# malb/m4ri

Measured on AMD Instinct MI355X. Metric: gf2_matmul_n3_equiv_bitops_per_sec, higher is better.
Workload: dtype u64; 1 GPU; mzd_mul 65536x65536x65536 (BASELINE.json configs[2]/[3]): Strassen-Winograd levels, the fused bottom ones by a rank-47 scheme of the 4 x 4 x 4 block product, over M4RM leaves; m=65536, l=65536, n=65536, input=splitmix64 seeds 3 (A), 4 (B), uniform bits, resident in HBM, strassen_levels=4, leaf_products_per_rank=2209, parallelism=1 GPU

## Files before the change

### m4ri_amd/csrc/scheme444.h

```cpp
#pragma once
#include <stdint.h>
#define SCHEME444_R 47
static constexpr uint16_t SCHEME444_U[SCHEME444_R] = {0x0101, 0x0808, 0x0d0d, 0x0e0e, 0x1000, 0x1001, 0x1010, 0x1110, 0x2d32, 0x3d32, 0x3d38, 0x3d3d, 0x3d3e, 0x5d08, 0x5d38, 0x5d58, 0x5d98, 0x6798, 0x6868, 0x6d38, 0x6e08, 0x7798, 0x8000, 0x8008, 0x8088, 0x8888, 0x9198, 0x9798, 0x9898, 0x9d98, 0xbd38, 0xcd01, 0xcd32, 0xcd98, 0xcdcd, 0xd000, 0xdd00, 0xddd0, 0xdddd, 0xe000, 0xe0e0, 0xe0ee, 0xee00, 0xf1fe, 0xf798, 0xfd32, 0xfe01};
static constexpr uint16_t SCHEME444_V[SCHEME444_R] = {0x0111, 0x1100, 0x0110, 0x0010, 0x0333, 0x0a14, 0xb1ac, 0xe7f9, 0x0927, 0x0777, 0x7700, 0x0a10, 0x0e10, 0xb1a0, 0x00f0, 0x7160, 0x0fff, 0x0aaa, 0x7760, 0x0aa0, 0xeef0, 0xe4ca, 0x3300, 0x4e50, 0x819f, 0xd7ca, 0xe1ff, 0x0060, 0xb1aa, 0x0660, 0x7d50, 0x011f, 0x00b0, 0xbb00, 0x0117, 0x0330, 0xb1af, 0x7e60, 0x0a17, 0x0030, 0x7d60, 0x0917, 0xe4fa, 0x0717, 0xee00, 0x0ee0, 0x0a1a};
static constexpr uint16_t SCHEME444_W[SCHEME444_R] = {0xbe5b, 0xb66b, 0xb1a0, 0xb158, 0xee0e, 0xbe5e, 0xbb0b, 0xbb5b, 0x4eae, 0x4ea4, 0xc66c, 0xb1a7, 0xb15f, 0xb6d0, 0xc628, 0xb11b, 0x0ee0, 0x8e68, 0xb16b, 0xc6a0, 0xb658, 0x8868, 0x6666, 0xb6b6, 0xbbbb, 0xbb6b, 0xb55b, 0x8268, 0xbd6b, 0x0aa0, 0xc6c6, 0xbe50, 0x4ea8, 0x0660, 0xb1ab, 0xa0a0, 0xb0b0, 0xb1b1, 0xb1a1, 0x28c8, 0xb1c1, 0xb151, 0xb858, 0xb15b, 0x8668, 0x4ea0, 0xbe58};
```

### m4ri_amd/csrc/scheme_passes.hip

```cpp
#include <hip/hip_runtime.h>
#include <cstdlib>
#include "gf2_internal.h"
#include "scheme444.h"

namespace {

constexpr int R444 = SCHEME444_R;

struct Tables { uint16_t m[3][3][50]; };
constexpr Tables make_tables() {
  Tables t{};
  constexpr uint16_t WG[3][7] = {{0x1, 0x2, 0xF, 0x8, 0xC, 0xD, 0x5}, {0x1, 0x4, 0x8, 0xF, 0x3, 0xB, 0xA}, {0xF, 0x1, 0x2, 0x4, 0xA, 0xE, 0xC}};
  for (int side = 0; side < 3; ++side) {
    t.m[0][side][0] = 1;
    for (int r = 0; r < 7; ++r) t.m[1][side][r] = WG[side][r];
    for (int r = 0; r < R444; ++r) t.m[2][side][r] = side == 0 ? SCHEME444_U[r] : side == 1 ? SCHEME444_V[r] : SCHEME444_W[r];
  }
  return t;
}
__constant__ Tables c_tab = make_tables();

struct Outer { int32_t r1, lv, side; };
__device__ __forceinline__ uint32_t outer_mask(const Outer &o, int r1) { return (uint32_t)c_tab.m[o.lv][o.side][r1]; }

template <int POS>
__device__ __forceinline__ uint32_t wave_union(uint32_t mine) {
  if (POS == 64) return __builtin_amdgcn_readfirstlane(mine);
  return __builtin_amdgcn_readfirstlane(mine) | __builtin_amdgcn_readlane(mine, 32);
}

template <int G, int POS>
__device__ __forceinline__ void form_top(const word *grid, uint32_t mine, int pp, word (&x)[16]) {
  constexpr int GD = 4 * G;
  const uint32_t both = wave_union<POS>(mine);
#pragma unroll
  for (int f = 0; f < 16; ++f) x[f] = 0;
#pragma unroll 1
  for (int c = 0; c < G * G; ++c) {
    if (!((both >> c) & 1)) continue;
    const word keep = (POS == 64 || ((mine >> c) & 1)) ? ~(word)0 : 0;
    const int i1 = c / G, j1 = c % G;
#pragma unroll
    for (int f = 0; f < 16; ++f) x[f] ^= grid[((4 * i1 + (f >> 2)) * GD + 4 * j1 + (f & 3)) * POS + pp] & keep;
  }
}

template <bool BSIDE>
__device__ __forceinline__ word inner_child(const word (&x)[16], int r2) {
  const uint16_t m = BSIDE ? SCHEME444_V[r2] : SCHEME444_U[r2];
  word v = 0;
#pragma unroll
  for (int f = 0; f < 16; ++f)
    if ((m >> f) & 1) v ^= x[f];
  return v;
}

template <int G, int POS, int UNITS, bool BSIDE>
__global__ __launch_bounds__(POS * UNITS) void scheme_down_kernel(const word *__restrict__ anc, int64_t p_stride, int64_t p_bs,
                                   word *__restrict__ child, int64_t c_bs,
                                   int64_t crows, int64_t cw, Outer o) {
  constexpr int GD = 4 * G, NB = GD * GD;
  __shared__ word grid[NB * POS];
  constexpr int units = UNITS;
  const int tid = threadIdx.x, pp = tid % POS, unit = tid / POS;
  const int64_t i = (int64_t)blockIdx.x * POS + pp, pi = blockIdx.y;
  const int64_t r = i / cw, w = i - r * cw;
  const word *p = anc + pi * p_bs + r * p_stride + w;
#pragma unroll 8
  for (int k = 0; k < (NB + UNITS - 1) / UNITS; ++k) {
    const int blk = k * UNITS + unit;
    if (NB % UNITS == 0 || blk < NB) grid[blk * POS + pp] = p[(int64_t)(blk / GD) * crows * p_stride + (int64_t)(blk % GD) * cw];
  }
  __syncthreads();
  word *out = child + pi * (int64_t)o.r1 * R444 * c_bs + r * cw + w;
  for (int r0 = 0; r0 < o.r1; r0 += units) {
    const int r1 = r0 + unit;
    const uint32_t mine = r1 < o.r1 ? outer_mask(o, r1) : 0u;
    word x[16];
    form_top<G, POS>(grid, mine, pp, x);
    if (r1 >= o.r1) continue;
    word *q = out + (int64_t)r1 * R444 * c_bs;
#pragma unroll
    for (int r2 = 0; r2 < R444; ++r2) q[(int64_t)r2 * c_bs] = inner_child<BSIDE>(x, r2);
  }
}

template <int G, int POS, int UNITS>
__global__ __launch_bounds__(POS * UNITS) void scheme_down_pack_kernel(const word *__restrict__ anc, int64_t p_stride, int64_t p_bs,
                                        uint32_t *__restrict__ a4, int64_t a4_bs,
                                        int64_t crows, int64_t cw, Outer o) {
  constexpr int GD = 4 * G, NB = GD * GD;
  __shared__ word grid[NB * POS];
  constexpr int units = UNITS;
  const int tid = threadIdx.x, pp = tid % POS, unit = tid / POS;
  const int64_t b = blockIdx.x, grp = b >> 7, xcd = b & 7, slot = (b >> 3) & 15;
  const int64_t wgroups = cw >> 4;
  const int64_t rb = (grp / wgroups) * 8 + xcd, wc = (grp % wgroups) * 16 + slot;
  if (rb * POS >= crows) return;
  const int64_t r = rb * POS + pp, pi = blockIdx.y;
  const word *p = anc + pi * p_bs + r * p_stride + wc;
#pragma unroll 8
  for (int k = 0; k < (NB + UNITS - 1) / UNITS; ++k) {
    const int blk = k * UNITS + unit;
    if (NB % UNITS == 0 || blk < NB) grid[blk * POS + pp] = p[(int64_t)(blk / GD) * crows * p_stride + (int64_t)(blk % GD) * cw];
  }
  __syncthreads();
  const uint32_t rot = (uint32_t)((r >> 6) & 3);
  uint32_t *out = a4 + pi * (int64_t)o.r1 * R444 * a4_bs + (2 * wc) * crows + r;
  for (int r0 = 0; r0 < o.r1; r0 += units) {
    const int r1 = r0 + unit;
    const uint32_t mine = r1 < o.r1 ? outer_mask(o, r1) : 0u;
    word x[16];
    form_top<G, POS>(grid, mine, pp, x);
    if (r1 >= o.r1) continue;
    uint32_t *q = out + (int64_t)r1 * R444 * a4_bs;
#pragma unroll
    for (int r2 = 0; r2 < R444; ++r2) {
      const word v = inner_child<false>(x, r2);
      uint32_t w0 = (uint32_t)v, w1 = (uint32_t)(v >> 32);
      w0 = __builtin_amdgcn_alignbyte(w0, w0, rot);
      w1 = __builtin_amdgcn_alignbyte(w1, w1, rot);
      uint32_t *oo = q + (int64_t)r2 * a4_bs;
      oo[0]     = w0;
      oo[crows] = w1;
    }
  }
}

template <int G, int POS, int UNITS, bool ACC>
__global__ __launch_bounds__(POS * UNITS) void scheme_up_kernel(const word *__restrict__ prod, int64_t p_bs,
                                 word *anc, int64_t o_stride, int64_t o_bs, int64_t crows, int64_t cw, Outer o) {
  constexpr int GD = 4 * G, NB = GD * GD;
  __shared__ unsigned long long g[NB * POS];
  constexpr int units = UNITS;
  const int tid = threadIdx.x, pp = tid % POS, unit = tid / POS;
  for (int k = tid; k < NB * POS; k += POS * UNITS) g[k] = 0;
  __syncthreads();
  const int64_t i = (int64_t)blockIdx.x * POS + pp, pi = blockIdx.y;
  const int64_t r = i / cw, w = i - r * cw;
  const word *q0 = prod + pi * (int64_t)o.r1 * R444 * p_bs + r * cw + w;
  for (int r1 = unit; r1 < o.r1; r1 += units) {
    const word *q = q0 + (int64_t)r1 * R444 * p_bs;
    word y[16];
#pragma unroll
    for (int f = 0; f < 16; ++f) y[f] = 0;
#pragma unroll
    for (int g0 = 0; g0 < R444; g0 += 8) {
      word v[8];
#pragma unroll
      for (int k = 0; k < 8; ++k)
        if (g0 + k < R444) v[k] = q[(int64_t)(g0 + k) * p_bs];
#pragma unroll
      for (int k = 0; k < 8; ++k)
        if (g0 + k < R444) {
          const uint16_t m = SCHEME444_W[g0 + k];
#pragma unroll
          for (int f = 0; f < 16; ++f)
            if ((m >> f) & 1) y[f] ^= v[k];
        }
    }
    const uint32_t mine = outer_mask(o, r1);
#pragma unroll 1
    for (int c = 0; c < G * G; ++c) {
      if (!((mine >> c) & 1)) continue;
      const int i1 = c / G, k1 = c % G;
#pragma unroll
      for (int f = 0; f < 16; ++f) atomicXor(&g[((4 * i1 + (f >> 2)) * GD + 4 * k1 + (f & 3)) * POS + pp], (unsigned long long)y[f]);
    }
  }
  __syncthreads();
  word *out = anc + pi * o_bs + r * o_stride + w;
#pragma unroll 4
  for (int k = 0; k < (NB + UNITS - 1) / UNITS; ++k) {
    const int blk = k * UNITS + unit;
    if (NB % UNITS != 0 && blk >= NB) continue;
    word *oo     = out + (int64_t)(blk / GD) * crows * o_stride + (int64_t)(blk % GD) * cw;
    const word v = g[blk * POS + pp];
    *oo          = ACC ? (*oo ^ v) : v;
  }
}

Outer outer_for(int levels, int side) { return Outer{levels == 4 ? R444 : levels == 3 ? 7 : 1, levels - 2, side}; }

constexpr int64_t MAX_GRID_Y = 65535;
constexpr int POS_B = 64;

}

extern "C" int gf2_scheme444_rank(void) { return R444; }

extern "C" int64_t gf2_scheme444_leaves(int levels) { return levels == 4 ? (int64_t)R444 * R444 : levels == 3 ? 7 * (int64_t)R444 : levels == 2 ? R444 : 0; }

extern "C" int gf2_scheme444_ok(int levels, int64_t a_rows, int64_t a_cw, int64_t b_rows, int64_t b_cw) {
  static const int sw = getenv("M4RI_AMD_SCHEME") ? atoi(getenv("M4RI_AMD_SCHEME")) : -1;
  if (sw == 0 || (sw == 4 && levels != 4) || (sw < 0 && R444 >= 49)) return 0;
  if (levels < 2 || levels > 4) return 0;
  if (a_rows <= 0 || b_rows <= 0 || a_rows % (levels == 2 ? 64 : 32) != 0 || a_cw % 16 != 0 || b_cw % POS_B != 0) return 0;
  if ((a_rows * a_cw) / 2 > 0x7fffffffLL || (b_rows * b_cw) / 32 > 0x7fffffffLL || (a_rows * b_cw) / 32 > 0x7fffffffLL) return 0;
  return 1;
}

template <typename F>
static void with_inner_grid(int levels, F &&f) {
  if (levels == 4) f(std::integral_constant<int, 4>{});
  else if (levels == 3) f(std::integral_constant<int, 2>{});
  else f(std::integral_constant<int, 1>{});
}

extern "C" hipError_t gf2_launch_scheme_down(hipStream_t s, int levels, int bside, const word *anc, int64_t p_stride, int64_t p_bs, word *child,
                                             int64_t nparents, int64_t crows, int64_t cw) {
  const int64_t c_bs = crows * cw;
  if (nparents * c_bs == 0) return hipSuccess;
  if (levels < 2 || levels > 4 || cw % 64 != 0) return hipErrorInvalidValue;
  const Outer o = outer_for(levels, bside ? 1 : 0);
  const int64_t leaves = gf2_scheme444_leaves(levels);
  for (int64_t p0 = 0; p0 < nparents; p0 += MAX_GRID_Y) {
    const int64_t np = nparents - p0 < MAX_GRID_Y ? nparents - p0 : MAX_GRID_Y;
    const word *an = anc + p0 * p_bs;
    word *ch       = child + p0 * leaves * c_bs;
    const dim3 g((unsigned)(c_bs / 64), (unsigned)np);
    with_inner_grid(levels, [&](auto G_) {
      constexpr int G = decltype(G_)::value, UNITS = G == 4 ? 8 : G == 2 ? 7 : 1;
      with_bool(bside, [&](auto BS) {
        hipLaunchKernelGGL((scheme_down_kernel<G, 64, UNITS, decltype(BS)::value>), g, dim3(64 * UNITS), 0, s, an, p_stride, p_bs, ch, c_bs, crows, cw, o);
      });
    });
  }
  return hipGetLastError();
}

extern "C" hipError_t gf2_launch_scheme_down_pack(hipStream_t s, int levels, const word *anc, int64_t p_stride, int64_t p_bs, word *a4,
                                                  int64_t nparents, int64_t crows, int64_t cw) {
  if (nparents * crows * cw == 0) return hipSuccess;
  const int pos = levels == 2 ? 64 : 32;
  if (levels < 2 || levels > 4 || crows % pos != 0 || cw % 16 != 0) return hipErrorInvalidValue;
  const Outer o = outer_for(levels, 0);
  const int64_t groups = ((crows / pos + 7) / 8) * (cw / 16);
  if (groups * 128 > 0x7fffffffLL) return hipErrorInvalidValue;
  const int64_t leaves = gf2_scheme444_leaves(levels);
  for (int64_t p0 = 0; p0 < nparents; p0 += MAX_GRID_Y) {
    const int64_t np = nparents - p0 < MAX_GRID_Y ? nparents - p0 : MAX_GRID_Y;
    const word *an = anc + p0 * p_bs;
    uint32_t *pk   = reinterpret_cast<uint32_t *>(a4) + p0 * leaves * crows * cw * 2;
    const dim3 g((unsigned)(groups * 128), (unsigned)np);
    with_inner_grid(levels, [&](auto G_) {
      constexpr int G = decltype(G_)::value, POS = G == 1 ? 64 : 32, UNITS = G == 1 ? 1 : 8;
      hipLaunchKernelGGL((scheme_down_pack_kernel<G, POS, UNITS>), g, dim3(POS * UNITS), 0, s, an, p_stride, p_bs, pk, crows * cw * 2, crows, cw, o);
    });
  }
  return hipGetLastError();
}

extern "C" hipError_t gf2_launch_scheme_up(hipStream_t s, int levels, int acc, const word *prod, word *anc, int64_t o_stride, int64_t o_bs,
                                           int64_t nparents, int64_t crows, int64_t cw) {
  const int64_t p_bs = crows * cw;
  if (nparents * p_bs == 0) return hipSuccess;
  if (levels < 2 || levels > 4 || cw % 64 != 0) return hipErrorInvalidValue;
  const Outer o = outer_for(levels, 2);
  const int pos = levels == 2 ? 64 : 32;
  const int64_t leaves = gf2_scheme444_leaves(levels);
  for (int64_t p0 = 0; p0 < nparents; p0 += MAX_GRID_Y) {
    const int64_t np = nparents - p0 < MAX_GRID_Y ? nparents - p0 : MAX_GRID_Y;
    const word *pr = prod + p0 * leaves * p_bs;
    word *an       = anc + p0 * o_bs;
    const dim3 g((unsigned)(p_bs / pos), (unsigned)np);
    with_inner_grid(levels, [&](auto G_) {
      constexpr int G = decltype(G_)::value, POS = G == 1 ? 64 : 32, UNITS = G == 1 ? 1 : 8;
      with_bool(acc, [&](auto ACC) {
        hipLaunchKernelGGL((scheme_up_kernel<G, POS, UNITS, decltype(ACC)::value>), g, dim3(POS * UNITS), 0, s, pr, p_bs, an, o_stride, o_bs, crows, cw, o);
      });
    });
  }
  return hipGetLastError();
}
```

Baseline: 11330000 billion bit-op/s.

## Use common-subexpression XOR programs for 4x4x4 scheme and wave-uniform outer loops

Replaces the naive per-output XOR accumulation of the rank-47 U, V and W^T maps with precomputed straight-line XOR programs that share intermediate sums. This cuts the XOR count in the down and up passes. The outer-rank loops are made wave-uniform and iterate only the set bits of the outer mask, which removes the wave-union masking. For POS=32, the pack and up kernels switch to 32-bit lanes so a full wave covers each block. The restructured lane/chunk addressing adds complexity and some correctness risk.

New measurement: 11380000 billion bit-op/s (median of 6 runs). No clear change (+0.4%).

```diff
diff --git a/m4ri_amd/csrc/scheme444.h b/m4ri_amd/csrc/scheme444.h
--- a/m4ri_amd/csrc/scheme444.h
+++ b/m4ri_amd/csrc/scheme444.h
@@ -4,3 +4,458 @@
 static constexpr uint16_t SCHEME444_U[SCHEME444_R] = {0x0101, 0x0808, 0x0d0d, 0x0e0e, 0x1000, 0x1001, 0x1010, 0x1110, 0x2d32, 0x3d32, 0x3d38, 0x3d3d, 0x3d3e, 0x5d08, 0x5d38, 0x5d58, 0x5d98, 0x6798, 0x6868, 0x6d38, 0x6e08, 0x7798, 0x8000, 0x8008, 0x8088, 0x8888, 0x9198, 0x9798, 0x9898, 0x9d98, 0xbd38, 0xcd01, 0xcd32, 0xcd98, 0xcdcd, 0xd000, 0xdd00, 0xddd0, 0xdddd, 0xe000, 0xe0e0, 0xe0ee, 0xee00, 0xf1fe, 0xf798, 0xfd32, 0xfe01};
 static constexpr uint16_t SCHEME444_V[SCHEME444_R] = {0x0111, 0x1100, 0x0110, 0x0010, 0x0333, 0x0a14, 0xb1ac, 0xe7f9, 0x0927, 0x0777, 0x7700, 0x0a10, 0x0e10, 0xb1a0, 0x00f0, 0x7160, 0x0fff, 0x0aaa, 0x7760, 0x0aa0, 0xeef0, 0xe4ca, 0x3300, 0x4e50, 0x819f, 0xd7ca, 0xe1ff, 0x0060, 0xb1aa, 0x0660, 0x7d50, 0x011f, 0x00b0, 0xbb00, 0x0117, 0x0330, 0xb1af, 0x7e60, 0x0a17, 0x0030, 0x7d60, 0x0917, 0xe4fa, 0x0717, 0xee00, 0x0ee0, 0x0a1a};
 static constexpr uint16_t SCHEME444_W[SCHEME444_R] = {0xbe5b, 0xb66b, 0xb1a0, 0xb158, 0xee0e, 0xbe5e, 0xbb0b, 0xbb5b, 0x4eae, 0x4ea4, 0xc66c, 0xb1a7, 0xb15f, 0xb6d0, 0xc628, 0xb11b, 0x0ee0, 0x8e68, 0xb16b, 0xc6a0, 0xb658, 0x8868, 0x6666, 0xb6b6, 0xbbbb, 0xbb6b, 0xb55b, 0x8268, 0xbd6b, 0x0aa0, 0xc6c6, 0xbe50, 0x4ea8, 0x0660, 0xb1ab, 0xa0a0, 0xb0b0, 0xb1b1, 0xb1a1, 0x28c8, 0xb1c1, 0xb151, 0xb858, 0xb15b, 0x8668, 0x4ea0, 0xbe58};
+
+#if defined(__HIPCC__)
+#define SCHEME444_FN __host__ __device__ __forceinline__
+#else
+#define SCHEME444_FN inline
+#endif
+
+#define SCHEME444_XORS_U 82
+template <typename T, typename Emit> SCHEME444_FN void scheme444_apply_u(const T (&x)[16], Emit &&emit) {
+  const T t16 = x[0] ^ x[8];
+  emit(0, t16);
+  const T t17 = x[3] ^ x[11];
+  emit(1, t17);
+  const T t18 = x[10] ^ x[11];
+  const T t19 = x[3] ^ t18;
+  const T t20 = x[0] ^ x[2];
+  const T t21 = x[8] ^ t20;
+  const T t22 = t19 ^ t21;
+  emit(2, t22);
+  const T t23 = x[1] ^ x[2];
+  const T t24 = t19 ^ t23;
+  const T t25 = x[9] ^ t24;
+  emit(3, t25);
+  emit(4, x[12]);
+  const T t26 = x[0] ^ x[12];
+  emit(5, t26);
+  const T t27 = x[4] ^ x[12];
+  emit(6, t27);
+  const T t28 = x[4] ^ x[8];
+  const T t29 = x[12] ^ t28;
+  emit(7, t29);
+  const T t30 = x[5] ^ x[13];
+  const T t31 = t28 ^ t30;
+  const T t32 = x[1] ^ t18;
+  const T t33 = t31 ^ t32;
+  emit(8, t33);
+  const T t34 = t29 ^ t30;
+  const T t35 = t34 ^ t32;
+  emit(9, t35);
+  const T t36 = t34 ^ t19;
+  emit(10, t36);
+  const T t37 = t20 ^ t36;
+  emit(11, t37);
+  const T t38 = t23 ^ t36;
+  emit(12, t38);
+  const T t39 = x[14] ^ t18;
+  const T t40 = x[3] ^ t39;
+  const T t41 = x[8] ^ x[12];
+  const T t42 = t40 ^ t41;
+  emit(13, t42);
+  const T t43 = t29 ^ t40;
+  const T t44 = x[5] ^ t43;
+  emit(14, t44);
+  const T t45 = x[6] ^ t43;
+  emit(15, t45);
+  const T t46 = x[3] ^ x[7];
+  const T t47 = t29 ^ t46;
+  const T t48 = t39 ^ t47;
+  emit(16, t48);
+  const T t49 = x[9] ^ x[13];
+  const T t50 = x[10] ^ x[14];
+  const T t51 = t49 ^ t50;
+  const T t52 = t46 ^ t51;
+  const T t53 = t28 ^ t52;
+  emit(17, t53);
+  const T t54 = x[6] ^ x[14];
+  const T t55 = t30 ^ t54;
+  const T t56 = t55 ^ t17;
+  emit(18, t56);
+  const T t57 = t40 ^ t31;
+  emit(19, t57);
+  const T t58 = t49 ^ t40;
+  emit(20, t58);
+  const T t59 = t51 ^ t47;
+  emit(21, t59);
+  emit(22, x[15]);
+  const T t60 = x[3] ^ x[15];
+  emit(23, t60);
+  const T t61 = x[15] ^ t46;
+  emit(24, t61);
+  const T t62 = x[11] ^ t61;
+  emit(25, t62);
+  const T t63 = t29 ^ t61;
+  emit(26, t63);
+  const T t64 = x[10] ^ t63;
+  const T t65 = x[9] ^ t64;
+  emit(27, t65);
+  const T t66 = t27 ^ t62;
+  emit(28, t66);
+  const T t67 = t18 ^ t63;
+  emit(29, t67);
+  const T t68 = x[15] ^ t36;
+  emit(30, t68);
+  const T t69 = x[15] ^ t39;
+  const T t70 = t69 ^ t16;
+  emit(31, t70);
+  const T t71 = x[1] ^ t69;
+  const T t72 = x[5] ^ t71;
+  const T t73 = t28 ^ t72;
+  emit(32, t73);
+  const T t74 = t39 ^ t61;
+  const T t75 = t28 ^ t74;
+  emit(33, t75);
+  const T t76 = x[6] ^ t74;
+  const T t77 = t21 ^ t76;
+  emit(34, t77);
+  const T t78 = x[14] ^ x[15];
+  const T t79 = x[12] ^ t78;
+  emit(35, t79);
+  const T t80 = t69 ^ t41;
+  emit(36, t80);
+  const T t81 = x[6] ^ t69;
+  const T t82 = t29 ^ t81;
+  const T t83 = x[7] ^ t82;
+  emit(37, t83);
+  const T t84 = x[6] ^ t39;
+  const T t85 = t63 ^ t84;
+  const T t86 = t20 ^ t85;
+  emit(38, t86);
+  const T t87 = x[13] ^ t78;
+  emit(39, t87);
+  const T t88 = x[7] ^ t55;
+  const T t89 = x[15] ^ t88;
+  emit(40, t89);
+  const T t90 = t61 ^ t23;
+  const T t91 = t55 ^ t90;
+  emit(41, t91);
+  const T t92 = t69 ^ t49;
+  emit(42, t92);
+  const T t93 = t54 ^ t90;
+  const T t94 = t34 ^ t93;
+  emit(43, t94);
+  const T t95 = t63 ^ t51;
+  emit(44, t95);
+  const T t96 = t34 ^ t71;
+  emit(45, t96);
+  const T t97 = t26 ^ t92;
+  emit(46, t97);
+}
+
+#define SCHEME444_XORS_V 80
+template <typename T, typename Emit> SCHEME444_FN void scheme444_apply_v(const T (&x)[16], Emit &&emit) {
+  const T t16 = x[4] ^ x[8];
+  const T t17 = x[0] ^ t16;
+  emit(0, t17);
+  const T t18 = x[8] ^ x[12];
+  emit(1, t18);
+  emit(2, t16);
+  emit(3, x[4]);
+  const T t19 = x[0] ^ x[1];
+  const T t20 = x[5] ^ x[9];
+  const T t21 = t16 ^ t20;
+  const T t22 = t19 ^ t21;
+  emit(4, t22);
+  const T t23 = x[4] ^ x[11];
+  const T t24 = x[9] ^ t23;
+  const T t25 = x[2] ^ t24;
+  emit(5, t25);
+  const T t26 = x[7] ^ x[15];
+  const T t27 = x[3] ^ t26;
+  const T t28 = x[13] ^ t18;
+  const T t29 = x[5] ^ t28;
+  const T t30 = t27 ^ t29;
+  const T t31 = x[2] ^ t30;
+  emit(6, t31);
+  const T t32 = x[9] ^ x[10];
+  const T t33 = x[5] ^ x[6];
+  const T t34 = x[13] ^ x[14];
+  const T t35 = t33 ^ t34;
+  const T t36 = t32 ^ t35;
+  const T t37 = t27 ^ t17;
+  const T t38 = t36 ^ t37;
+  emit(7, t38);
+  const T t39 = x[2] ^ t19;
+  const T t40 = x[8] ^ x[11];
+  const T t41 = x[5] ^ t40;
+  const T t42 = t39 ^ t41;
+  emit(8, t42);
+  const T t43 = t16 ^ t39;
+  const T t44 = t33 ^ t32;
+  const T t45 = t43 ^ t44;
+  emit(9, t45);
+  const T t46 = t32 ^ t34;
+  const T t47 = t18 ^ t46;
+  emit(10, t47);
+  emit(11, t24);
+  const T t48 = t32 ^ t23;
+  emit(12, t48);
+  const T t49 = t26 ^ t29;
+  emit(13, t49);
+  const T t50 = x[7] ^ t33;
+  const T t51 = x[4] ^ t50;
+  emit(14, t51);
+  const T t52 = t18 ^ t35;
+  emit(15, t52);
+  const T t53 = x[7] ^ x[11];
+  const T t54 = t53 ^ t45;
+  const T t55 = x[3] ^ t54;
+  emit(16, t55);
+  const T t56 = x[1] ^ x[3];
+  const T t57 = t53 ^ t20;
+  const T t58 = t56 ^ t57;
+  emit(17, t58);
+  const T t59 = t18 ^ t36;
+  emit(18, t59);
+  emit(19, t57);
+  const T t60 = t23 ^ t36;
+  const T t61 = t26 ^ t60;
+  emit(20, t61);
+  const T t62 = x[1] ^ t27;
+  const T t63 = x[6] ^ t34;
+  const T t64 = x[10] ^ t63;
+  const T t65 = t62 ^ t64;
+  emit(21, t65);
+  const T t66 = x[9] ^ t28;
+  emit(22, t66);
+  const T t67 = x[14] ^ t32;
+  const T t68 = x[6] ^ t67;
+  const T t69 = t23 ^ t68;
+  emit(23, t69);
+  const T t70 = t27 ^ t43;
+  emit(24, t70);
+  const T t71 = t18 ^ t68;
+  const T t72 = t62 ^ t71;
+  emit(25, t72);
+  const T t73 = t35 ^ t70;
+  emit(26, t73);
+  emit(27, t33);
+  const T t74 = t62 ^ t29;
+  emit(28, t74);
+  emit(29, t44);
+  const T t75 = x[11] ^ x[12];
+  const T t76 = t16 ^ t64;
+  const T t77 = t75 ^ t76;
+  emit(30, t77);
+  const T t78 = x[3] ^ t43;
+  emit(31, t78);
+  const T t79 = x[4] ^ x[5];
+  const T t80 = x[7] ^ t79;
+  emit(32, t80);
+  const T t81 = x[11] ^ x[15];
+  const T t82 = t81 ^ t66;
+  emit(33, t82);
+  emit(34, t43);
+  emit(35, t21);
+  const T t83 = t39 ^ t30;
+  emit(36, t83);
+  const T t84 = t36 ^ t75;
+  emit(37, t84);
+  const T t85 = t39 ^ t24;
+  emit(38, t85);
+  emit(39, t79);
+  const T t86 = x[10] ^ t35;
+  const T t87 = x[11] ^ t86;
+  const T t88 = t18 ^ t87;
+  emit(40, t88);
+  const T t89 = x[11] ^ t43;
+  emit(41, t89);
+  const T t90 = t62 ^ t86;
+  const T t91 = x[4] ^ t90;
+  emit(42, t91);
+  const T t92 = t32 ^ t43;
+  emit(43, t92);
+  const T t93 = t81 ^ t46;
+  emit(44, t93);
+  const T t94 = t44 ^ t53;
+  emit(45, t94);
+  const T t95 = t24 ^ t56;
+  emit(46, t95);
+}
+
+#define SCHEME444_XORS_WT 118
+template <typename T, typename Load> SCHEME444_FN void scheme444_apply_wt(Load &&ld, T (&y)[16]) {
+  const T p0 = ld(0);
+  const T p1 = ld(1);
+  const T p2 = ld(2);
+  const T p3 = ld(3);
+  const T p4 = ld(4);
+  const T p5 = ld(5);
+  const T p6 = ld(6);
+  const T p7 = ld(7);
+  const T t47 = p0 ^ p5;
+  const T p8 = ld(8);
+  const T p9 = ld(9);
+  const T p10 = ld(10);
+  const T p11 = ld(11);
+  const T p12 = ld(12);
+  const T p13 = ld(13);
+  const T p14 = ld(14);
+  const T p15 = ld(15);
+  const T p16 = ld(16);
+  const T p17 = ld(17);
+  const T p18 = ld(18);
+  const T p19 = ld(19);
+  const T p20 = ld(20);
+  const T p21 = ld(21);
+  const T p22 = ld(22);
+  const T p23 = ld(23);
+  const T t48 = p11 ^ p23;
+  const T t49 = p10 ^ p22;
+  const T t50 = p14 ^ p19;
+  const T t51 = p22 ^ t47;
+  const T t52 = p17 ^ p21;
+  const T p24 = ld(24);
+  const T p25 = ld(25);
+  const T p26 = ld(26);
+  const T p27 = ld(27);
+  const T p28 = ld(28);
+  const T p29 = ld(29);
+  const T p30 = ld(30);
+  const T p31 = ld(31);
+  const T t53 = p7 ^ p25;
+  const T t54 = p18 ^ p28;
+  const T t55 = p12 ^ p26;
+  const T t56 = p6 ^ p24;
+  const T t57 = t53 ^ t56;
+  const T t58 = p4 ^ p30;
+  const T t59 = t58 ^ t50;
+  const T t60 = p8 ^ t58;
+  const T t61 = t48 ^ t60;
+  const T t62 = p16 ^ t53;
+  const T t63 = p12 ^ t61;
+  const T t64 = p5 ^ t63;
+  const T t65 = p23 ^ p24;
+  const T t66 = t49 ^ t64;
+  const T t67 = p9 ^ t66;
+  const T p32 = ld(32);
+  const T p33 = ld(33);
+  const T p34 = ld(34);
+  const T p35 = ld(35);
+  const T p36 = ld(36);
+  const T p37 = ld(37);
+  const T p38 = ld(38);
+  const T p39 = ld(39);
+  const T t68 = p34 ^ t54;
+  const T t69 = p1 ^ t68;
+  const T t70 = p8 ^ p32;
+  const T t71 = p37 ^ p38;
+  const T t72 = p2 ^ t71;
+  const T t73 = p36 ^ t48;
+  const T t74 = t72 ^ t73;
+  const T t75 = p33 ^ t49;
+  const T t76 = p35 ^ t74;
+  const T t77 = p4 ^ p39;
+  const T t78 = p1 ^ t75;
+  const T t79 = p30 ^ p39;
+  const T t80 = p13 ^ t79;
+  const T t81 = t54 ^ t78;
+  const T p40 = ld(40);
+  const T p41 = ld(41);
+  const T p42 = ld(42);
+  const T p43 = ld(43);
+  const T p44 = ld(44);
+  const T p45 = ld(45);
+  const T p46 = ld(46);
+  const T t82 = p46 ^ t47;
+  const T t83 = p43 ^ t55;
+  const T t84 = p20 ^ t82;
+  const T t85 = p15 ^ t83;
+  const T t86 = t57 ^ t85;
+  const T t87 = p13 ^ t84;
+  const T t88 = p31 ^ t87;
+  const T t89 = t69 ^ t86;
+  const T t90 = p17 ^ p44;
+  const T t91 = p3 ^ p42;
+  const T t92 = p9 ^ p45;
+  const T t93 = t70 ^ t92;
+  const T t94 = p40 ^ p41;
+  const T t95 = p27 ^ t90;
+  const T t96 = t88 ^ t91;
+  const T t97 = p16 ^ t93;
+  const T t98 = p21 ^ t95;
+  const T t99 = t94 ^ t96;
+  const T t100 = p29 ^ t97;
+  const T t101 = t89 ^ t99;
+  const T t102 = t76 ^ t100;
+  const T t103 = p23 ^ t88;
+  const T t104 = t59 ^ t103;
+  const T t105 = p10 ^ t98;
+  const T t106 = p24 ^ t102;
+  const T t107 = t57 ^ t100;
+  const T t108 = t76 ^ t101;
+  const T t109 = t78 ^ t104;
+  const T t110 = p11 ^ t94;
+  const T t111 = t89 ^ t61;
+  const T t112 = t71 ^ t89;
+  const T t113 = p31 ^ p42;
+  const T t114 = t82 ^ t107;
+  const T t115 = p25 ^ t98;
+  const T t116 = t72 ^ t110;
+  const T t117 = t70 ^ t89;
+  const T t118 = t110 ^ t112;
+  const T t119 = t77 ^ t114;
+  const T t120 = t91 ^ t77;
+  const T t121 = p26 ^ t97;
+  const T t122 = t85 ^ t96;
+  const T t123 = p28 ^ t109;
+  const T t124 = t50 ^ t115;
+  const T t125 = t98 ^ t99;
+  const T t126 = t75 ^ t124;
+  const T t127 = p37 ^ t122;
+  const T t128 = p19 ^ p40;
+  const T t129 = t83 ^ t81;
+  const T t130 = p36 ^ t127;
+  const T t131 = t59 ^ t105;
+  const T t132 = t62 ^ t129;
+  const T t133 = t69 ^ t106;
+  const T t134 = t77 ^ t108;
+  const T t135 = t113 ^ t119;
+  const T t136 = p3 ^ t86;
+  const T t137 = t93 ^ t59;
+  const T t138 = t84 ^ t105;
+  const T t139 = t90 ^ t123;
+  const T t140 = t68 ^ t136;
+  const T t141 = p7 ^ t130;
+  const T t142 = p14 ^ t117;
+  const T t143 = t79 ^ t125;
+  const T t144 = t126 ^ t133;
+  const T t145 = t80 ^ t128;
+  const T t146 = t121 ^ t139;
+  const T t147 = t65 ^ t141;
+  const T t148 = t120 ^ t142;
+  const T t149 = p34 ^ t106;
+  const T t150 = t145 ^ t149;
+  const T t151 = t107 ^ t109;
+  const T t152 = p28 ^ t135;
+  const T t153 = p0 ^ t118;
+  const T t154 = t108 ^ t131;
+  const T t155 = t138 ^ t148;
+  const T t156 = t95 ^ t151;
+  const T t157 = t74 ^ t101;
+  const T t158 = t132 ^ t143;
+  const T t159 = p22 ^ t134;
+  const T t160 = t116 ^ t140;
+  const T t161 = t52 ^ t152;
+  const T t162 = p41 ^ t147;
+  const T t163 = t111 ^ t51;
+  const T t164 = t49 ^ t137;
+  y[0] = t153;
+  y[1] = t163;
+  y[2] = t67;
+  y[3] = t155;
+  y[4] = t162;
+  y[5] = t144;
+  y[6] = t158;
+  y[7] = t150;
+  y[8] = t160;
+  y[9] = t156;
+  y[10] = t146;
+  y[11] = t161;
+  y[12] = t157;
+  y[13] = t159;
+  y[14] = t164;
+  y[15] = t154;
+}
diff --git a/m4ri_amd/csrc/scheme_passes.hip b/m4ri_amd/csrc/scheme_passes.hip
--- a/m4ri_amd/csrc/scheme_passes.hip
+++ b/m4ri_amd/csrc/scheme_passes.hip
@@ -23,45 +23,37 @@
 struct Outer { int32_t r1, lv, side; };
 __device__ __forceinline__ uint32_t outer_mask(const Outer &o, int r1) { return (uint32_t)c_tab.m[o.lv][o.side][r1]; }
 
-template <int POS>
-__device__ __forceinline__ uint32_t wave_union(uint32_t mine) {
-  if (POS == 64) return __builtin_amdgcn_readfirstlane(mine);
-  return __builtin_amdgcn_readfirstlane(mine) | __builtin_amdgcn_readlane(mine, 32);
-}
-
-template <int G, int POS>
-__device__ __forceinline__ void form_top(const word *grid, uint32_t mine, int pp, word (&x)[16]) {
-  constexpr int GD = 4 * G;
-  const uint32_t both = wave_union<POS>(mine);
+constexpr int WAVE = 64;
+
+template <int POS> struct Elem { typedef word type; };
+template <> struct Elem<32> { typedef uint32_t type; };
+
+__device__ __forceinline__ int wave_uniform(int v) { return __builtin_amdgcn_readfirstlane(v); }
+
+template <int G>
+__device__ __forceinline__ int block_at(int c, int f) {
+  return ((4 * (c / G) + (f >> 2)) * (4 * G) + 4 * (c % G) + (f & 3)) * WAVE;
+}
+
+template <int G, typename T>
+__device__ __forceinline__ void form_top(const T *cell, uint32_t mask, T (&x)[16]) {
 #pragma unroll
   for (int f = 0; f < 16; ++f) x[f] = 0;
 #pragma unroll 1
-  for (int c = 0; c < G * G; ++c) {
-    if (!((both >> c) & 1)) continue;
-    const word keep = (POS == 64 || ((mine >> c) & 1)) ? ~(word)0 : 0;
-    const int i1 = c / G, j1 = c % G;
+  for (uint32_t m = mask; m; m &= m - 1) {
+    const int c = __builtin_ctz(m);
 #pragma unroll
-    for (int f = 0; f < 16; ++f) x[f] ^= grid[((4 * i1 + (f >> 2)) * GD + 4 * j1 + (f & 3)) * POS + pp] & keep;
-  }
-}
-
-template <bool BSIDE>
-__device__ __forceinline__ word inner_child(const word (&x)[16], int r2) {
-  const uint16_t m = BSIDE ? SCHEME444_V[r2] : SCHEME444_U[r2];
-  word v = 0;
-#pragma unroll
-  for (int f = 0; f < 16; ++f)
-    if ((m >> f) & 1) v ^= x[f];
-  return v;
+    for (int f = 0; f < 16; ++f) x[f] ^= cell[block_at<G>(c, f)];
+  }
 }
 
 template <int G, int POS, int UNITS, bool BSIDE>
 __global__ __launch_bounds__(POS * UNITS) void scheme_down_kernel(const word *__restrict__ anc, int64_t p_stride, int64_t p_bs,
                                    word *__restrict__ child, int64_t c_bs,
                                    int64_t crows, int64_t cw, Outer o) {
+  static_assert(POS == WAVE, "a unit of this kernel is a wave");
   constexpr int GD = 4 * G, NB = GD * GD;
   __shared__ word grid[NB * POS];
-  constexpr int units = UNITS;
   const int tid = threadIdx.x, pp = tid % POS, unit = tid / POS;
   const int64_t i = (int64_t)blockIdx.x * POS + pp, pi = blockIdx.y;
   const int64_t r = i / cw, w = i - r * cw;
@@ -73,15 +65,13 @@
   }
   __syncthreads();
   word *out = child + pi * (int64_t)o.r1 * R444 * c_bs + r * cw + w;
-  for (int r0 = 0; r0 < o.r1; r0 += units) {
-    const int r1 = r0 + unit;
-    const uint32_t mine = r1 < o.r1 ? outer_mask(o, r1) : 0u;
+  for (int r1 = wave_uniform(unit); r1 < o.r1; r1 += UNITS) {
     word x[16];
-    form_top<G, POS>(grid, mine, pp, x);
-    if (r1 >= o.r1) continue;
+    form_top<G>(grid + pp, outer_mask(o, r1), x);
     word *q = out + (int64_t)r1 * R444 * c_bs;
-#pragma unroll
-    for (int r2 = 0; r2 < R444; ++r2) q[(int64_t)r2 * c_bs] = inner_child<BSIDE>(x, r2);
+    const auto store = [&](int r2, word v) { q[(int64_t)r2 * c_bs] = v; };
+    if (BSIDE) scheme444_apply_v(x, store);
+    else scheme444_apply_u(x, store);
   }
 }
 
@@ -89,9 +79,10 @@
 __global__ __launch_bounds__(POS * UNITS) void scheme_down_pack_kernel(const word *__restrict__ anc, int64_t p_stride, int64_t p_bs,
                                         uint32_t *__restrict__ a4, int64_t a4_bs,
                                         int64_t crows, int64_t cw, Outer o) {
-  constexpr int GD = 4 * G, NB = GD * GD;
-  __shared__ word grid[NB * POS];
-  constexpr int units = UNITS;
+  typedef typename Elem<POS>::type T;
+  constexpr int GD = 4 * G, NB = GD * GD, WAVES = POS * UNITS / WAVE;
+  static_assert((POS * UNITS) % WAVE == 0 && POS * sizeof(word) == WAVE * sizeof(T), "a block is WAVE elements");
+  __shared__ T grid[NB * WAVE];
   const int tid = threadIdx.x, pp = tid % POS, unit = tid / POS;
   const int64_t b = blockIdx.x, grp = b >> 7, xcd = b & 7, slot = (b >> 3) & 15;
   const int64_t wgroups = cw >> 4;
@@ -102,74 +93,66 @@
 #pragma unroll 8
   for (int k = 0; k < (NB + UNITS - 1) / UNITS; ++k) {
     const int blk = k * UNITS + unit;
-    if (NB % UNITS == 0 || blk < NB) grid[blk * POS + pp] = p[(int64_t)(blk / GD) * crows * p_stride + (int64_t)(blk % GD) * cw];
+    if (NB % UNITS != 0 && blk >= NB) continue;
+    const word v = p[(int64_t)(blk / GD) * crows * p_stride + (int64_t)(blk % GD) * cw];
+    if (POS == WAVE) grid[blk * WAVE + pp] = (T)v;
+    else {
+      grid[blk * WAVE + pp]       = (T)v;
+      grid[blk * WAVE + POS + pp] = (T)(v >> 32);
+    }
   }
   __syncthreads();
   const uint32_t rot = (uint32_t)((r >> 6) & 3);
-  uint32_t *out = a4 + pi * (int64_t)o.r1 * R444 * a4_bs + (2 * wc) * crows + r;
-  for (int r0 = 0; r0 < o.r1; r0 += units) {
-    const int r1 = r0 + unit;
-    const uint32_t mine = r1 < o.r1 ? outer_mask(o, r1) : 0u;
-    word x[16];
-    form_top<G, POS>(grid, mine, pp, x);
-    if (r1 >= o.r1) continue;
+  const int lane = tid % WAVE, chunk = POS == WAVE ? 0 : lane / POS;
+  uint32_t *out = a4 + pi * (int64_t)o.r1 * R444 * a4_bs + (2 * wc + chunk) * crows + r;
+  for (int r1 = wave_uniform(tid / WAVE); r1 < o.r1; r1 += WAVES) {
+    T x[16];
+    form_top<G>(grid + lane, outer_mask(o, r1), x);
     uint32_t *q = out + (int64_t)r1 * R444 * a4_bs;
-#pragma unroll
-    for (int r2 = 0; r2 < R444; ++r2) {
-      const word v = inner_child<false>(x, r2);
-      uint32_t w0 = (uint32_t)v, w1 = (uint32_t)(v >> 32);
-      w0 = __builtin_amdgcn_alignbyte(w0, w0, rot);
-      w1 = __builtin_amdgcn_alignbyte(w1, w1, rot);
+    scheme444_apply_u(x, [&](int r2, T v) {
       uint32_t *oo = q + (int64_t)r2 * a4_bs;
-      oo[0]     = w0;
-      oo[crows] = w1;
-    }
-  }
-}
+      const uint32_t w0 = (uint32_t)v;
+      oo[0] = __builtin_amdgcn_alignbyte(w0, w0, rot);
+      if (POS == WAVE) {
+        const uint32_t w1 = (uint32_t)((word)v >> 32);
+        oo[crows] = __builtin_amdgcn_alignbyte(w1, w1, rot);
+      }
+    });
+  }
+}
+
+__device__ __forceinline__ void lds_xor(uint32_t *a, uint32_t v) { atomicXor(reinterpret_cast<unsigned int *>(a), (unsigned int)v); }
+__device__ __forceinline__ void lds_xor(word *a, word v) { atomicXor(reinterpret_cast<unsigned long long *>(a), (unsigned long long)v); }
 
 template <int G, int POS, int UNITS, bool ACC>
 __global__ __launch_bounds__(POS * UNITS) void scheme_up_kernel(const word *__restrict__ prod, int64_t p_bs,
                                  word *anc, int64_t o_stride, int64_t o_bs, int64_t crows, int64_t cw, Outer o) {
-  constexpr int GD = 4 * G, NB = GD * GD;
-  __shared__ unsigned long long g[NB * POS];
-  constexpr int units = UNITS;
+  typedef typename Elem<POS>::type T;
+  constexpr int GD = 4 * G, NB = GD * GD, WAVES = POS * UNITS / WAVE, E = sizeof(word) / sizeof(T);
+  static_assert((POS * UNITS) % WAVE == 0 && POS * E == WAVE, "a block is WAVE elements");
+  typedef T __attribute__((may_alias)) Cell;
+  __shared__ word g[NB * POS];
   const int tid = threadIdx.x, pp = tid % POS, unit = tid / POS;
   for (int k = tid; k < NB * POS; k += POS * UNITS) g[k] = 0;
   __syncthreads();
-  const int64_t i = (int64_t)blockIdx.x * POS + pp, pi = blockIdx.y;
-  const int64_t r = i / cw, w = i - r * cw;
-  const word *q0 = prod + pi * (int64_t)o.r1 * R444 * p_bs + r * cw + w;
-  for (int r1 = unit; r1 < o.r1; r1 += units) {
-    const word *q = q0 + (int64_t)r1 * R444 * p_bs;
-    word y[16];
+  const int64_t i0 = (int64_t)blockIdx.x * POS, pi = blockIdx.y;
+  const int64_t r = i0 / cw, w0 = i0 - r * cw;
+  const int lane = tid % WAVE;
+  const T *q0 = reinterpret_cast<const T *>(prod + pi * (int64_t)o.r1 * R444 * p_bs + r * cw + w0) + lane;
+  Cell *cell  = reinterpret_cast<Cell *>(g) + lane;
+  for (int r1 = wave_uniform(tid / WAVE); r1 < o.r1; r1 += WAVES) {
+    const T *q = q0 + (int64_t)r1 * R444 * p_bs * E;
+    T y[16];
+    scheme444_apply_wt([&](int) { const T v = *q; q += p_bs * E; return v; }, y);
+#pragma unroll 1
+    for (uint32_t m = outer_mask(o, r1); m; m &= m - 1) {
+      const int c = __builtin_ctz(m);
 #pragma unroll
-    for (int f = 0; f < 16; ++f) y[f] = 0;
-#pragma unroll
-    for (int g0 = 0; g0 < R444; g0 += 8) {
-      word v[8];
-#pragma unroll
-      for (int k = 0; k < 8; ++k)
-        if (g0 + k < R444) v[k] = q[(int64_t)(g0 + k) * p_bs];
-#pragma unroll
-      for (int k = 0; k < 8; ++k)
-        if (g0 + k < R444) {
-          const uint16_t m = SCHEME444_W[g0 + k];
-#pragma unroll
-          for (int f = 0; f < 16; ++f)
-            if ((m >> f) & 1) y[f] ^= v[k];
-        }
+      for (int f = 0; f < 16; ++f) lds_xor(cell + block_at<G>(c, f), y[f]);
     }
-    const uint32_t mine = outer_mask(o, r1);
-#pragma unroll 1
-    for (int c = 0; c < G * G; ++c) {
-      if (!((mine >> c) & 1)) continue;
-      const int i1 = c / G, k1 = c % G;
-#pragma unroll
-      for (int f = 0; f < 16; ++f) atomicXor(&g[((4 * i1 + (f >> 2)) * GD + 4 * k1 + (f & 3)) * POS + pp], (unsigned long long)y[f]);
-    }
-  }
-  __syncthreads();
-  word *out = anc + pi * o_bs + r * o_stride + w;
+  }
+  __syncthreads();
+  word *out = anc + pi * o_bs + r * o_stride + w0 + pp;
 #pragma unroll 4
   for (int k = 0; k < (NB + UNITS - 1) / UNITS; ++k) {
     const int blk = k * UNITS + unit;
```
